# jlvdb/yet_another_wizz

Measured on AMD Instinct MI355X. Metric: candidate pairs/s, higher is better.
Workload: dtype f64

## Files before the change

yet_another_wizz_amd/csrc/yawhip_band32.inc:

```
namespace {

constexpr int B32_WAVES_PLAIN = 7;
constexpr int B32_WAVES_BIG = 6;
constexpr int B32_WAVES_W = 5;
constexpr int B32_WAVES_W1 = 5;
constexpr int B32_WAVES_LT = 1;
constexpr int band32_min_waves(int R, int CAP, bool WEIGHTED, int NE, bool UNI) {
    if (NE == 2 && UNI) {
        if (WEIGHTED) return R == 1 ? B32_WAVES_W1 : B32_WAVES_W;
        return CAP >= B32_CAP_BIG ? B32_WAVES_BIG : B32_WAVES_PLAIN;
    }
    return NE == 2 && !WEIGHTED ? B32_WAVES_LT : 1;
}

template <int R, int CAP, bool WEIGHTED, int NE, bool MERGED, bool UNI>
__global__ __launch_bounds__(64, band32_min_waves(R, CAP, WEIGHTED, NE, UNI))
void YAW_B32_NAME(const DevTab *__restrict__ tabs, const Item *__restrict__ items, int n_bins,
                  const double *__restrict__ t, const float *__restrict__ thr32,
                  const double *__restrict__ rwin_k, const float *__restrict__ ucap,
                  unsigned flush_mask, int swap,
                  unsigned long long *__restrict__ out_counts,
                  double *__restrict__ partials,
                  unsigned long long *__restrict__ counters, unsigned long long seg_cap) {
    static_assert(NE >= 2 && NE <= 4, "edges per bin");
    constexpr int CH = YAW_B32_CH;
    constexpr bool PAIRS = R == 1 && CH == 1;
    constexpr int NS = PAIRS ? 2 : R;
    static_assert(CH == 1 || CH == 3, "chunks per round");
    static_assert(CAP % 4 == 0, "stage capacity");
    using HistT = typename std::conditional<WEIGHTED, double, unsigned int>::type;
    constexpr int NC = NE == 2 ? 1 : NE;
    constexpr int NF = NE - 1;
    constexpr int TW = thr32_width(NE);
    constexpr bool LANE_THR = MERGED && !UNI;
    extern __shared__ __attribute__((aligned(16))) unsigned char lds_dyn[];
    const int nkb = MERGED ? n_bins : 1;
    const int nslots = nkb * NF;
    unsigned char *p = lds_dyn;
    constexpr unsigned COLB = (CAP + 4) * 4;
    float *stage = reinterpret_cast<float *>(p); p += (size_t)3 * COLB;
    double *sw = reinterpret_cast<double *>(p); if (WEIGHTED) p += (size_t)(CAP + 4) * 8;
    HistT *hist = reinterpret_cast<HistT *>(p); p += (size_t)nslots * sizeof(HistT);
    p = reinterpret_cast<unsigned char *>(((size_t)p + 15) & ~(size_t)15);
    float *sthr = reinterpret_cast<float *>(p);
    const int lane = threadIdx.x;
    const unsigned a_stage = (unsigned)(size_t)(lds_byte *)reinterpret_cast<unsigned char *>(stage);
    const unsigned a_sw = (unsigned)(size_t)(lds_byte *)reinterpret_cast<unsigned char *>(sw);
    const unsigned a_hist = (unsigned)(size_t)(lds_byte *)reinterpret_cast<unsigned char *>(hist);

    const TicketMap tmap = ticket_map(counters, seg_cap);
    const unsigned long long n_kept = tmap.n_kept;
    for (int e = lane; e < nslots; e += 64) hist[e] = HistT(0);
    if (LANE_THR)
        for (int e = lane; e < n_bins * TW; e += 64) sthr[e] = thr32[e];
    unsigned round_no = 0;
    for (unsigned long long v = blockIdx.x;; v += gridDim.x) {
        if ((v >> 3) >= tmap.per_xcd) break;
        const unsigned long long ticket = tmap.ticket(v);
        if (ticket >= n_kept) continue;
        const Item it = items[ticket];
        const int o = item_orient(it), islot = item_slot(it);
        const DevTab cl = tabs[swap ? o : 3 + o], cs = tabs[swap ? 3 + o : o];
        const int kfix = MERGED ? 0 : islot % n_bins;
        const float rwin = (float)(rwin_k[kfix] * 1.000001 + 4e-7);

        int win = 0;
        int64_t win_off = 0;
        int64_t cb[CH];
        int cn[CH], co[CH];
        int nch = 0;
        auto next_round = [&]() {
            nch = 0;
            int used = 0;
#pragma unroll
            for (int c = 0; c < CH; ++c) {
                cb[c] = 0; cn[c] = 0; co[c] = 0;
                if (win < it.nwin && nch == c) {
                    const int64_t wb = win == 0 ? it.b0[0] : (win == 1 ? it.b0[1] : it.b0[2]);
                    const int64_t rem = (int64_t)(win == 0 ? it.nb[0] : (win == 1 ? it.nb[1] : it.nb[2])) - win_off;
                    if (rem + 1 <= (int64_t)(CAP - used)) {
                        cb[c] = wb + win_off; cn[c] = (int)rem; co[c] = used;
                        used += ((int)rem + 1 + 3) & ~3;
                        ++win; win_off = 0; ++nch;
                    } else if (c == 0) {
                        cb[c] = wb + win_off; cn[c] = CAP - 4; co[c] = 0;
                        used = CAP;
                        win_off += CAP - 4; ++nch;
                    }
                }
            }
        };
        auto issue_round = [&]() {
#pragma unroll
            for (int c = 0; c < CH; ++c) {
                if (c < nch) {
                    const gf32p gx = cs.qx + cb[c], gy = cs.qy + cb[c], gz = cs.qz + cb[c];
                    const unsigned a_c = a_stage + ((unsigned)co[c] << 2);
#pragma unroll
                    for (int k = 0; k < (CAP + 255) / 256; ++k) {
                        const unsigned e = (unsigned)(k * 256 + 4 * lane);
                        if (e < (unsigned)cn[c]) {
                            __builtin_amdgcn_global_load_lds(gx + e, lds_ptr(a_c + k * 1024), 16, 0, 0);
                            __builtin_amdgcn_global_load_lds(gy + e, lds_ptr(a_c + COLB + k * 1024), 16, 0, 0);
                            __builtin_amdgcn_global_load_lds(gz + e, lds_ptr(a_c + 2 * COLB + k * 1024), 16, 0, 0);
                        }
                    }
                    if (WEIGHTED && cs.w) {
#pragma unroll
                        for (int k = 0; k < (CAP + 127) / 128; ++k) {
                            const unsigned e = (unsigned)(k * 128 + 2 * lane);
                            if (e < (unsigned)cn[c])
                                __builtin_amdgcn_global_load_lds(cs.w + cb[c] + e, lds_ptr(a_sw + ((unsigned)co[c] << 3) + k * 1024), 16, 0, 0);
                        }
                    }
                }
            }
        };
        __syncthreads();
        next_round();
        issue_round();
        f32x2 ax2[R / 2 > 0 ? R / 2 : 1], ay2[R / 2 > 0 ? R / 2 : 1], az2[R / 2 > 0 ? R / 2 : 1];
        float ax[R], ay[R], az[R];
        int kb[R];
        double aw_own[R];
        int lane_obj = lane;
        int n_own = (int)it.na - lane * R;
        n_own = n_own < 0 ? 0 : (n_own > R ? R : n_own);
#pragma unroll
        for (int r = 0; r < R; ++r) {
            const bool have = r < n_own;
            const unsigned ic = have ? (unsigned)(lane * R + r) : 0u;
            ax[r] = have ? (cl.qx + it.a0)[ic] : PAD_COORD32;
            ay[r] = have ? (cl.qy + it.a0)[ic] : PAD_COORD32;
            az[r] = have ? (cl.qz + it.a0)[ic] : PAD_COORD32;
            kb[r] = MERGED ? (have ? (cl.k + it.a0)[ic] : 0) : 0;
            if constexpr (WEIGHTED) aw_own[r] = (cl.w && have) ? (cl.w + it.a0)[ic] : 1.0;
        }
        float th[R][TW];
        {
            const float *row = LANE_THR ? nullptr : thr32 + (size_t)kfix * TW;
#pragma unroll
            for (int r = 0; r < R; ++r)
#pragma unroll
                for (int q = 0; q < TW; ++q) th[r][q] = LANE_THR ? sthr[kb[r] * TW + q] : row[q];
        }
        float klo, khi;
        {
            const int last_r = n_own > 0 ? n_own - 1 : 0;
            float u_first = cl.axis == 0 ? ax[0] : (cl.axis == 1 ? ay[0] : az[0]), u_last = u_first;
#pragma unroll
            for (int r = 1; r < R; ++r)
                if (r == last_r) u_last = cl.axis == 0 ? ax[r] : (cl.axis == 1 ? ay[r] : az[r]);
            klo = u_first - rwin;
            khi = u_last + rwin;
            const float cap_c = ucap[2 * kfix], cap_s = ucap[2 * kfix + 1];
            if (cap_s > 0.0f) {
                klo = cap_lo32(u_first, cap_c, cap_s);
                khi = cap_hi32(u_last, cap_c, cap_s);
            }
        }
        if constexpr (R >= 2) {
#pragma unroll
            for (int h = 0; h < R / 2; ++h) {
                ax2[h] = f32x2{ax[2 * h], ax[2 * h + 1]}; ay2[h] = f32x2{ay[2 * h], ay[2 * h + 1]}; az2[h] = f32x2{az[2 * h], az[2 * h + 1]};
            }
        }
        f32x2 nc2[R / 2 > 0 ? R / 2 : 1];
#pragma unroll
        for (int h = 0; h < R / 2; ++h) nc2[h] = f32x2{-th[2 * h][0], -th[2 * h + 1][0]};
        unsigned int cnt[R][NC];
        double acc[R][NC];
#pragma unroll
        for (int r = 0; r < R; ++r)
#pragma unroll
            for (int c = 0; c < NC; ++c) { cnt[r][c] = 0u; acc[r][c] = 0.0; }
        unsigned int nev = 0;
        constexpr bool HALF = R == 1 && CH == 1;
        const double pair_mult = HALF && (it.pad_ & 1) ? 2.0 : 1.0;
        auto flush_lanes = [&]() {
#pragma unroll
            for (int r = 0; r < R; ++r) {
#pragma unroll
                for (int f = 0; f < NF; ++f) {
                    const unsigned cell = a_hist + (unsigned)((kb[r] * NF + f) * (int)sizeof(HistT));
                    if constexpr (WEIGHTED) {
                        const double vsum = NE == 2 ? acc[r][0] : acc[r][f + 1] - acc[r][f];
                        const double aw = aw_own[r];
                        if (vsum != 0.0)
                            (void)__hip_atomic_fetch_add((__attribute__((address_space(3))) double *)(size_t)cell, HALF ? aw * vsum * pair_mult : aw * vsum,
                                                         __ATOMIC_RELAXED, __HIP_MEMORY_SCOPE_WORKGROUP);
                    } else {
                        const unsigned int c = (NE == 2 ? cnt[r][0] : cnt[r][f + 1] - cnt[r][f]) << (HALF ? (it.pad_ & 1) : 0);
                        if (c)
                            (void)__hip_atomic_fetch_add((__attribute__((address_space(3))) unsigned int *)(size_t)cell, c,
                                                         __ATOMIC_RELAXED, __HIP_MEMORY_SCOPE_WORKGROUP);
                    }
                }
#pragma unroll
                for (int c = 0; c < NC; ++c) { cnt[r][c] = 0u; acc[r][c] = 0.0; }
            }
        };
        auto flush_counts = [&]() {
            flush_lanes();
            __syncthreads();
            for (int idx = lane; idx < nslots; idx += 64) {
                const unsigned int c = (unsigned int)hist[idx];
                hist[idx] = HistT(0);
                if (c) atomicAdd(&out_counts[(int64_t)islot * nslots + idx], (unsigned long long)c);
            }
        };

        const bool single_window = it.nwin == 1 && it.nb[0] + 1 <= CAP;
        for (;; ++round_no) {
            asm volatile("s_waitcnt vmcnt(0)" ::: "memory");
            __syncthreads();
            if (lane < nch) {
                int at = co[0] + cn[0];
                if constexpr (CH > 1) at = lane == 0 ? at : (lane == 1 ? co[1] + cn[1] : co[CH - 1] + cn[CH - 1]);
                stage[at] = PAD_COORD32; stage[COLB / 4 + at] = PAD_COORD32; stage[2 * (COLB / 4) + at] = PAD_COORD32;
                if (WEIGHTED) sw[at] = 0.0;
                if constexpr (PAIRS) {
                    stage[at + 1] = PAD_COORD32; stage[COLB / 4 + at + 1] = PAD_COORD32; stage[2 * (COLB / 4) + at + 1] = PAD_COORD32;
                    if (WEIGHTED) sw[at + 1] = 0.0;
                }
            }
            if (WEIGHTED && !cs.w) {
#pragma unroll
                for (int c = 0; c < CH; ++c)
                    if (c < nch)
                        for (int e = lane; e < cn[c]; e += 64) sw[co[c] + e] = 1.0;
            }
            __syncthreads();
            unsigned a_key[CH], a_sent[CH], ql[CH], qh[CH];
            int n_max = 1;
#pragma unroll
            for (int c = 0; c < CH; ++c) {
                a_key[c] = a_stage + COLB * (unsigned)cl.axis + ((unsigned)co[c] << 2);
                a_sent[c] = a_key[c] + ((unsigned)cn[c] << 2);
                ql[c] = qh[c] = a_key[c] - 4u;
                n_max = cn[c] > n_max ? cn[c] : n_max;
            }
            for (unsigned step = 4u << (31 - __builtin_clz(n_max)); step >= 4u; step >>= 1) {
#pragma unroll
                for (int c = 0; c < CH; ++c) {
                    if (c < nch) {
                        const unsigned pl = ql[c] + step, ph = qh[c] + step;
                        const float kl = *(const __attribute__((address_space(3))) float *)(size_t)(pl < a_sent[c] ? pl : a_sent[c]);
                        const float kh = *(const __attribute__((address_space(3))) float *)(size_t)(ph < a_sent[c] ? ph : a_sent[c]);
                        ql[c] = kl < klo ? pl : ql[c];
                        qh[c] = kh <= khi ? ph : qh[c];
                    }
                }
            }
#pragma unroll
            for (int c = 0; c < CH; ++c) {
            if (c < nch) {
            const int n = cn[c];
            int lo = (int)((ql[c] + 4u - a_key[c]) >> 2), hi = (int)((qh[c] + 4u - a_key[c]) >> 2);
            if (n_own == 0) lo = hi = n;
            if constexpr (R == 1 && CH == 1) {
                if (it.pad_ & 1) {
                    const int own = n_own > 0 ? (int)((long long)(cl.pos3 + it.a0)[lane] - (long long)cb[c]) + 1 : n;
                    lo = own > lo ? own : lo;
                    lo = lo > hi ? hi : lo;
                }
            }
            int len = hi - lo;
            unsigned stride = PAIRS ? 8u : 4u;
            nev += (unsigned int)(len * n_own);
            if (single_window) {
                const unsigned long long act = __builtin_amdgcn_ballot_w64(len > 0);
                const int first = act ? __builtin_ctzll(act) : 0, span = act ? 64 - __builtin_clzll(act) - first : 64;
                if (span <= 32) {
                    const int sh = span <= 8 ? 3 : (span <= 16 ? 2 : 1);
                    const bool idle = (lane >> sh) >= span;
                    const int src = idle ? first : first + (lane >> sh);
                    const int part = lane & ((1 << sh) - 1);
                    if constexpr (R >= 2) {
#pragma unroll
                        for (int h = 0; h < R / 2; ++h) {
                            ax2[h] = f32x2{__shfl(ax2[h].x, src, 64), __shfl(ax2[h].y, src, 64)};
                            ay2[h] = f32x2{__shfl(ay2[h].x, src, 64), __shfl(ay2[h].y, src, 64)};
                            az2[h] = f32x2{__shfl(az2[h].x, src, 64), __shfl(az2[h].y, src, 64)};
                        }
                    }
#pragma unroll
                    for (int r = 0; r < R; ++r) {
                        if constexpr (R < 2) { ax[r] = __shfl(ax[r], src, 64); ay[r] = __shfl(ay[r], src, 64); az[r] = __shfl(az[r], src, 64); }
                        if constexpr (MERGED) kb[r] = __shfl(kb[r], src, 64);
                        if constexpr (WEIGHTED) aw_own[r] = __shfl(aw_own[r], src, 64);
                        if constexpr (LANE_THR) {
#pragma unroll
                            for (int q = 0; q < TW; ++q) th[r][q] = sthr[kb[r] * TW + q];
                        }
                    }
                    if constexpr (LANE_THR && NE == 2) {
#pragma unroll
                        for (int h = 0; h < R / 2; ++h) nc2[h] = f32x2{-th[2 * h][0], -th[2 * h + 1][0]};
                    }
                    n_own = __shfl(n_own, src, 64);
                    lane_obj = src;
                    const int lo_s = __shfl(lo, src, 64), len_s = __shfl(len, src, 64);
                    if constexpr (PAIRS) {
                        const int pairs_s = (len_s + 1) >> 1;
                        lo = idle ? n : lo_s + 2 * part;
                        len = !idle && pairs_s > part ? ((pairs_s - part + (1 << sh) - 1) >> sh) << 1 : 0;
                        stride = 8u << sh;
                    } else {
                        lo = idle ? n : lo_s + part;
                        len = !idle && len_s > part ? (len_s - part + (1 << sh) - 1) >> sh : 0;
                        stride = 4u << sh;
                    }
                }
            }
            const int steps = wave_max_nonneg(PAIRS ? (len + 1) >> 1 : len);

            const unsigned a_chunk = a_stage + ((unsigned)co[c] << 2);
            unsigned cur = a_chunk + ((unsigned)lo << 2);
            const unsigned last = a_chunk + ((unsigned)n << 2);
            auto eval_entry = [&](const unsigned a16) {
                struct { float x, y, z; } en, en1;
                en.x = *(const __attribute__((address_space(3))) float *)(size_t)a16;
                en.y = *(const __attribute__((address_space(3))) float *)(size_t)(a16 + COLB);
                en.z = *(const __attribute__((address_space(3))) float *)(size_t)(a16 + 2 * COLB);
                if constexpr (PAIRS) {
                    en1.x = *(const __attribute__((address_space(3))) float *)(size_t)(a16 + 4u);
                    en1.y = *(const __attribute__((address_space(3))) float *)(size_t)(a16 + 4u + COLB);
                    en1.z = *(const __attribute__((address_space(3))) float *)(size_t)(a16 + 4u + 2 * COLB);
                }
                double ewi[NS];
                const unsigned a_w = ((a16 - a_stage) << 1) + a_sw;
                ewi[0] = WEIGHTED ? lds_f64(a_w) : 1.0;
                if constexpr (PAIRS) ewi[1] = WEIGHTED ? lds_f64(a_w + 8u) : 1.0;
                else {
#pragma unroll
                    for (int i = 1; i < NS; ++i) ewi[i] = ewi[0];
                }
                float s32[NS];
                if constexpr (PAIRS) {
                    const f32x2 dx = ax[0] - f32x2{en.x, en1.x}, dy = ay[0] - f32x2{en.y, en1.y}, dz = az[0] - f32x2{en.z, en1.z};
                    f32x2 sq;
                    if constexpr (NE == 2) {
                        const f32x2 nc = f32x2{-th[0][0], -th[0][0]};
                        sq = __builtin_elementwise_fma(dz, dz, __builtin_elementwise_fma(dy, dy, __builtin_elementwise_fma(dx, dx, nc)));
                    } else sq = __builtin_elementwise_fma(dz, dz, __builtin_elementwise_fma(dy, dy, dx * dx));
                    s32[0] = sq.x; s32[1] = sq.y;
                } else if constexpr (R >= 2) {
#pragma unroll
                    for (int h = 0; h < R / 2; ++h) {
                        const f32x2 dx = ax2[h] - en.x, dy = ay2[h] - en.y, dz = az2[h] - en.z;
                        f32x2 sq;
                        if constexpr (NE == 2) sq = __builtin_elementwise_fma(dz, dz, __builtin_elementwise_fma(dy, dy, __builtin_elementwise_fma(dx, dx, nc2[h])));
                        else sq = __builtin_elementwise_fma(dz, dz, __builtin_elementwise_fma(dy, dy, dx * dx));
                        s32[2 * h] = sq.x; s32[2 * h + 1] = sq.y;
                    }
                } else {
                    const float dx = ax[0] - en.x, dy = ay[0] - en.y, dz = az[0] - en.z;
                    if constexpr (NE == 2) s32[0] = __builtin_fmaf(dz, dz, __builtin_fmaf(dy, dy, __builtin_fmaf(dx, dx, -th[0][0])));
                    else s32[0] = __builtin_fmaf(dz, dz, __builtin_fmaf(dy, dy, dx * dx));
                }
                unsigned long long unc_mask[NS];
                unsigned long long any_mask = 0ull;
#pragma unroll
                for (int i = 0; i < NS; ++i) {
                    const int r = PAIRS ? 0 : i;
                    const double ew = ewi[i];
                    if constexpr (NE == 2) {
                        const float q = __builtin_fabsf(s32[i]);
                        const bool in = q < th[r][1];
                        unc_mask[i] = __builtin_amdgcn_ballot_w64(q < th[r][2]) & ~__builtin_amdgcn_ballot_w64(in);
                        if constexpr (WEIGHTED) acc[r][0] = __builtin_fma(in ? 1.0 : 0.0, ew, acc[r][0]);
                        else cnt[r][0] += in ? 1u : 0u;
                    } else {
                        unc_mask[i] = 0ull;
#pragma unroll
                        for (int e = 0; e < NE; ++e) {
                            const bool le = s32[i] < th[r][2 * e];
                            unc_mask[i] |= __builtin_amdgcn_ballot_w64(s32[i] <= th[r][2 * e + 1]) & ~__builtin_amdgcn_ballot_w64(le);
                            if constexpr (WEIGHTED) acc[r][e] = __builtin_fma(le ? 1.0 : 0.0, ew, acc[r][e]);
                            else cnt[r][e] += le ? 1u : 0u;
                        }
                    }
                    any_mask |= unc_mask[i];
                }
                if (any_mask != 0ull) {
#pragma unroll
                    for (int i = 0; i < NS; ++i) {
                        const int r = PAIRS ? 0 : i;
                        const unsigned eidx = ((a16 - a_chunk) >> 2) + (PAIRS ? (unsigned)i : 0u);
                        const double ew = ewi[i];
                        if (((unc_mask[i] >> lane) & 1ull) && eidx < (unsigned)n && r < n_own) {
                            const ExactEval<NE> ev = band32_exact<NE>(cl.x, cl.y, cl.z, it.a0 + lane_obj * R + r, cs.x, cs.y, cs.z,
                                                                      cs.idx ? (int64_t)cs.idx[cb[c] + eidx] : cb[c] + (int64_t)eidx,
                                                                      t + (size_t)(MERGED ? kb[r] : kfix) * NE,
                                                                      counters + EXACT_EVAL_CTR(0) + CTR_SLOT_WORDS * (ticket & (EVAL_SLOTS - 1)));
                            const double sd = ev.s;
                            if constexpr (NE == 2) {
                                const bool in = sd > ev.th[0] && sd <= ev.th[1];
                                if constexpr (WEIGHTED) acc[r][0] += in ? ew : 0.0;
                                else cnt[r][0] += in ? 1u : 0u;
                            } else {
#pragma unroll
                                for (int e = 0; e < NE; ++e) {
                                    const bool open = !(s32[i] < th[r][2 * e]) && s32[i] <= th[r][2 * e + 1];
                                    const bool le = open && sd <= ev.th[e];
                                    if constexpr (WEIGHTED) acc[r][e] += le ? ew : 0.0;
                                    else cnt[r][e] += le ? 1u : 0u;
                                }
                            }
                        }
                    }
                }
            };
            constexpr int UNROLL = 1;
            for (int s = 0; s < steps; s += UNROLL) {
#pragma unroll
                for (int uu = 0; uu < UNROLL; ++uu) {
                    const unsigned at = cur + stride * (unsigned)uu;
                    eval_entry(at < last ? at : last);
                }
                cur += stride * UNROLL;
            }
            }
            }
            if (!WEIGHTED && (round_no & flush_mask) == flush_mask) flush_counts();
            if (win >= it.nwin) break;
            __syncthreads();
            next_round();
            issue_round();
        }
        ++round_no;
        if constexpr (WEIGHTED) {
            flush_lanes();
            __syncthreads();
            for (int idx = lane; idx < nslots; idx += 64) {
                partials[(int64_t)it.pot * nslots + idx] = (double)hist[idx];
                hist[idx] = HistT(0);
            }
        } else {
            flush_counts();
        }
        nev = wave_sum_lane63(nev);
        if (lane == 63 && nev) atomicAdd(&counters[BAND_ENTRY_CTR(ticket & (EVAL_SLOTS - 1))], (unsigned long long)nev);
    }
}

}

namespace yawhip_detail {

hipError_t YAW_B32_LAUNCH(const CountLaunch &L, bool wgt, int32_t *variant) {
    const std::pair<int, int> stage{L.R, L.cap};
    const std::pair<bool, bool> rows{L.merged, L.uni};
    const dim3 band_grid(L.band_grid), wave(64);
    return pick<Bool<false>, Bool<true>>(wgt, [&](auto w) {
        return pick<Int<4>, Int<3>, Int<2>>(L.n_edges, [&](auto ne) {
            return pick<Rows<true, false>, Rows<true, true>, Rows<false, true>>(rows, [&](auto r) {
                return pick<Stage<4, B32_CAP_BIG>, Stage<2, B32_CAP_BIG>, Stage<2, B32_CAP>, Stage<1, B32_CAP>>(stage, [&](auto s) {
                    using S = decltype(s);
                    using M = decltype(r);
                    *variant = variant_code(YAW_B32_CH == 1 ? VF_BAND32_ONE : VF_BAND32, S::R, S::CAP, w, ne, M::MERGED, M::UNI);
                    return launch(YAW_B32_NAME<S::R, S::CAP, w, ne, M::MERGED, M::UNI>, band_grid, wave, L.lds, L.stream, L.d_tabs,
                                  L.d_items, L.n_bins, L.d_t, L.d_thr32, L.d_rwin, L.d_ucap, L.flush_mask, L.swap ? 1 : 0,
                                  L.d_counts, L.d_partials, L.d_ctr, L.seg_cap);
                });
            });
        });
    });
}

}
```

yet_another_wizz_amd/csrc/yawhip_count_kernels.h:

```cpp
#ifndef YAWHIP_COUNT_KERNELS_H
#define YAWHIP_COUNT_KERNELS_H
#include <hip/hip_runtime.h>

#include <algorithm>
#include <cmath>
#include <cstddef>
#include <cstdint>

#include "yawhip_internal.h"

#pragma GCC visibility push(hidden)

namespace yawhip_detail {

constexpr int WG = 256;
constexpr int STAGE = 256;
constexpr int MSTAGE = 64;
constexpr int MAX_EDGES = 512;
constexpr int BAND_MIN_STREAM_RUN = 64;
constexpr int64_t SYNC_GRID_MIN_ITEMS = 400000;
constexpr int MAX_STRIP_REACH = 12;

constexpr double FILTER_GUARD = 8.0 * 5.9604644775390625e-8;

inline double sep_angle(double rwin) { return 2.0 * std::asin(std::min(1.0, 0.5 * (rwin + 2e-9))); }

constexpr int EVAL_SLOTS = 256;
constexpr int BUILD_WG = 1024;
constexpr int BUILD_WG_SMALL = 256;
inline int build_wg_for(int64_t n_pot) { return n_pot / 256 <= 4096 ? BUILD_WG_SMALL : BUILD_WG; }
constexpr int BUILD_PREFIX_LDS = 1024;
constexpr int ITEM_SEGS = 8;

constexpr int BCAP = 192;
constexpr int BCAP_MID = 288;
constexpr int B32_CAP = 320;
constexpr int B32_CAP_BIG = 512;

constexpr double BAND32_GUARD_SQRT = 2.1e-7;
__host__ __device__ constexpr int thr32_width(int ne) { return ne == 2 ? 4 : 2 * ne; }
__host__ __device__ constexpr int fine32_width(int n_edges) { return 4 + 2 * n_edges; }

constexpr int REDUCE_CHUNK = 32;
constexpr int TAIL_WG = 256;
constexpr unsigned TAIL_MAX_GRID = 64;
constexpr double CLOCK_MS = 1.0e-5;

int band_lds_fixed(int cap);
__host__ __device__ inline bool band_small_hist(bool weighted, int nslots, int hp) { return (size_t)nslots * hp * (weighted ? 8 : 4) <= 512; }
__host__ __device__ inline size_t band_lds_dynamic(bool weighted, bool need_thr, int nkb, int n_edges, int hp, int cap, int thr_rows) {
    const int nslots = nkb * (n_edges - 1);
    return (weighted ? (size_t)(cap + 2) * 8 : 0) + (need_thr ? (size_t)thr_rows * n_edges * sizeof(double) : 0) +
           (band_small_hist(weighted, nslots, hp) ? 0 : (size_t)nslots * hp * (weighted ? 8 : 4)) + 16;
}
__host__ __device__ inline size_t band32_lds(bool weighted, int cap, int nslots, int thr_rows, int ne) {
    return (size_t)3 * (cap + 4) * 4 + (weighted ? (size_t)(cap + 4) * 8 : 0) + (size_t)nslots * (weighted ? 8 : 4) +
           (size_t)thr_rows * thr32_width(ne) * 4 + 32;
}
__host__ __device__ inline size_t band32_fine_lds(bool weighted, int cap, int nslots, int rows, int n_edges) {
    return (size_t)3 * (cap + 4) * 4 + (weighted ? (size_t)(cap + 2) * 8 : 0) + (size_t)nslots * (weighted ? 8 : 4) + 64 * 8 +
           (size_t)rows * fine32_width(n_edges) * 4 + 48;
}
size_t count_lds(bool weighted, bool priv, int n_edges);
size_t merged_stage_lds();
size_t merged_lds(bool weighted, int bins, int n_edges);

constexpr int CTR_KEPT = 0, CTR_T_BUILD = 1, CTR_T_COUNTED = 2, CTR_T_TAIL = 3, CTR_TICKET = 4, CTR_DONE = 6;
constexpr int CTR_SLOT_WORDS = 8;
template <typename I> __host__ __device__ constexpr auto BAND_ENTRY_CTR(I i) { return 8 + CTR_SLOT_WORDS * i; }
template <typename I> __host__ __device__ constexpr auto EXACT_EVAL_CTR(I i) { return 9 + CTR_SLOT_WORDS * i; }
template <typename I> __host__ __device__ constexpr auto TILE_PAIR_CTR(I i) { return 10 + CTR_SLOT_WORDS * i; }
__host__ __device__ constexpr int ITEM_SEG_CTR(int seg) { return 12 + CTR_SLOT_WORDS * seg; }
__host__ __device__ constexpr int SEG_EXIT_CTR(int seg) { return ITEM_SEG_CTR(seg) + 1; }
constexpr int N_CTR = 8 + CTR_SLOT_WORDS * EVAL_SLOTS;
static_assert(BAND_ENTRY_CTR(0) % CTR_SLOT_WORDS == 0 && EXACT_EVAL_CTR(0) % CTR_SLOT_WORDS == 1 && TILE_PAIR_CTR(0) % CTR_SLOT_WORDS == 2 &&
                  ITEM_SEG_CTR(0) % CTR_SLOT_WORDS == 4 && SEG_EXIT_CTR(0) % CTR_SLOT_WORDS == 5,
              "the segment words and the per-slot words take different places of a slot's line");
static_assert(CTR_DONE < BAND_ENTRY_CTR(0) && ITEM_SEGS <= EVAL_SLOTS && TILE_PAIR_CTR(EVAL_SLOTS - 1) < N_CTR, "counter block");

enum class CountFamily : int32_t { PLAIN, LEAN, BAND64, BAND32, BAND32_FINE };
struct CountLaunch {
    hipStream_t stream = nullptr;
    CountFamily family = CountFamily::PLAIN;
    int R = 0, cap = 0, band_ne = 0;
    bool merged = false, uni = false, nf1 = false, filter = false, priv = false, one_chunk = false;
    unsigned build_grid = 0, build_wg = 0, band_grid = 0;
    int64_t n_pot = 0;
    int64_t n_items = 0;
    int64_t n_build_jobs = 0;
    int64_t n_oslots = 0;
    int64_t tile = 0, slab = 0, n_chunks = 0;
    size_t lds = 0;
    unsigned flush_mask = 0;
    int batch_log2 = 0, hp_shift = 0, n_bins = 0, n_edges = 0, reach = 0;
    bool swap = false, triple = false;
    unsigned long long seg_cap = 0;
    double rwin_max = 0.0, cap_c = 1.0, cap_s = 0.0;
    CatView c1{}, c2{};
    const DevTab *d_tabs = nullptr;
    const int32_t *d_jobs = nullptr;
    const int64_t *d_prefix = nullptr, *d_cprefix = nullptr;
    const double *d_t = nullptr, *d_rwin = nullptr;
    const float *d_dthr = nullptr, *d_ucap = nullptr, *d_thr32 = nullptr;
    Item *d_items = nullptr;
    unsigned char *d_kept = nullptr;
    unsigned long long *d_ctr = nullptr, *d_counts = nullptr;
    double *d_partials = nullptr, *d_chunk_sums = nullptr, *d_sums = nullptr;
};

hipError_t launch_build_strips(const CountLaunch &L);
hipError_t launch_build_windows(const CountLaunch &L);
hipError_t launch_build_whole(const CountLaunch &L);
hipError_t launch_item_work(const CountLaunch &L, int slots_per_job, unsigned long long *job_work);
hipError_t launch_count(const CountLaunch &L, bool weighted, int32_t *variant);
hipError_t launch_plain(const CountLaunch &L, bool weighted, int32_t *variant);
hipError_t launch_lean(const CountLaunch &L, bool weighted, int32_t *variant);
hipError_t launch_band64(const CountLaunch &L, bool weighted, int32_t *variant);
hipError_t launch_band32(const CountLaunch &L, bool weighted, int32_t *variant);
hipError_t launch_band32_one(const CountLaunch &L, bool weighted, int32_t *variant);
hipError_t launch_fine(const CountLaunch &L, bool weighted, int32_t *variant);
hipError_t launch_reduce_chunks(const CountLaunch &L);
hipError_t launch_reduce_slots(const CountLaunch &L);
hipError_t launch_counts_to_double(const CountLaunch &L, int64_t n_out);
hipError_t launch_call_tail(hipStream_t stream, unsigned char *dev, unsigned char *host, unsigned n_copy, unsigned n_clean,
                            unsigned long long seq);

}

#pragma GCC visibility pop
#endif
```

Measured before the change: 34220000 billion.

## Hand-code unweighted two-slot band32 inner loop in packed-f32 inline asm

For unweighted two-edge, two-object (R=2) band32 kernels without per-lane thresholds, the per-entry classify step is replaced by inline assembly. It uses packed f32 subtract/FMA, scalar-mask comparisons and carry-add counting, and splits classification from the rare exact-evaluation path. When there is one chunk per round, the loop walks the staged entries downward from the top using a clamped subtract. It pads four leading LDS slots with PAD_COORD32 so out-of-range reads hit sentinels, and reserves 48 extra LDS bytes for this. The goal is fewer VALU/SALU instructions and less loop-control overhead per candidate. The cost is brittle asm, a trap if the LDS base is not the expected offset, and more LDS use.

```diff
diff --git a/yet_another_wizz_amd/csrc/yawhip_band32.inc b/yet_another_wizz_amd/csrc/yawhip_band32.inc
--- a/yet_another_wizz_amd/csrc/yawhip_band32.inc
+++ b/yet_another_wizz_amd/csrc/yawhip_band32.inc
@@ -37,8 +37,12 @@
     const int nkb = MERGED ? n_bins : 1;
     const int nslots = nkb * NF;
     unsigned char *p = lds_dyn;
-    constexpr unsigned COLB = (CAP + 4) * 4;
-    float *stage = reinterpret_cast<float *>(p); p += (size_t)3 * COLB;
+    constexpr bool SLOT_TRIP = NE == 2 && !WEIGHTED && R == 2 && !LANE_THR;
+    constexpr bool DOWN = SLOT_TRIP && CH == 1;
+    constexpr int LEAD = DOWN ? 4 : 0;
+    constexpr unsigned COLB = (CAP + 4 + LEAD) * 4;
+    float *const stage_lead = reinterpret_cast<float *>(p);
+    float *stage = stage_lead + LEAD; p += (size_t)3 * COLB;
     double *sw = reinterpret_cast<double *>(p); if (WEIGHTED) p += (size_t)(CAP + 4) * 8;
     HistT *hist = reinterpret_cast<HistT *>(p); p += (size_t)nslots * sizeof(HistT);
     p = reinterpret_cast<unsigned char *>(((size_t)p + 15) & ~(size_t)15);
@@ -51,6 +55,10 @@
     const TicketMap tmap = ticket_map(counters, seg_cap);
     const unsigned long long n_kept = tmap.n_kept;
     for (int e = lane; e < nslots; e += 64) hist[e] = HistT(0);
+    if constexpr (DOWN) {
+        if (a_stage != 4u * LEAD) __builtin_trap();
+        if (lane < LEAD) { stage_lead[lane] = PAD_COORD32; stage_lead[COLB / 4 + lane] = PAD_COORD32; stage_lead[2 * (COLB / 4) + lane] = PAD_COORD32; }
+    }
     if (LANE_THR)
         for (int e = lane; e < n_bins * TW; e += 64) sthr[e] = thr32[e];
     unsigned round_no = 0;
@@ -266,6 +274,7 @@
                 }
             }
             int len = hi - lo;
+            int top = hi - 1;
             unsigned stride = PAIRS ? 8u : 4u;
             nev += (unsigned int)(len * n_own);
             if (single_window) {
@@ -308,6 +317,7 @@
                         stride = 8u << sh;
                     } else {
                         lo = idle ? n : lo_s + part;
+                        top = lo_s + len_s - 1 - part;
                         len = !idle && len_s > part ? (len_s - part + (1 << sh) - 1) >> sh : 0;
                         stride = 4u << sh;
                     }
@@ -318,7 +328,7 @@
             const unsigned a_chunk = a_stage + ((unsigned)co[c] << 2);
             unsigned cur = a_chunk + ((unsigned)lo << 2);
             const unsigned last = a_chunk + ((unsigned)n << 2);
-            auto eval_entry = [&](const unsigned a16) {
+            auto classify_entry = [&](const unsigned a16, unsigned long long (&unc_mask)[NS], float (&s32)[NS], double (&ewi)[NS]) {
                 struct { float x, y, z; } en, en1;
                 en.x = *(const __attribute__((address_space(3))) float *)(size_t)a16;
                 en.y = *(const __attribute__((address_space(3))) float *)(size_t)(a16 + COLB);
@@ -328,7 +338,6 @@
                     en1.y = *(const __attribute__((address_space(3))) float *)(size_t)(a16 + 4u + COLB);
                     en1.z = *(const __attribute__((address_space(3))) float *)(size_t)(a16 + 4u + 2 * COLB);
                 }
-                double ewi[NS];
                 const unsigned a_w = ((a16 - a_stage) << 1) + a_sw;
                 ewi[0] = WEIGHTED ? lds_f64(a_w) : 1.0;
                 if constexpr (PAIRS) ewi[1] = WEIGHTED ? lds_f64(a_w + 8u) : 1.0;
@@ -336,7 +345,6 @@
 #pragma unroll
                     for (int i = 1; i < NS; ++i) ewi[i] = ewi[0];
                 }
-                float s32[NS];
                 if constexpr (PAIRS) {
                     const f32x2 dx = ax[0] - f32x2{en.x, en1.x}, dy = ay[0] - f32x2{en.y, en1.y}, dz = az[0] - f32x2{en.z, en1.z};
                     f32x2 sq;
@@ -359,7 +367,6 @@
                     if constexpr (NE == 2) s32[0] = __builtin_fmaf(dz, dz, __builtin_fmaf(dy, dy, __builtin_fmaf(dx, dx, -th[0][0])));
                     else s32[0] = __builtin_fmaf(dz, dz, __builtin_fmaf(dy, dy, dx * dx));
                 }
-                unsigned long long unc_mask[NS];
                 unsigned long long any_mask = 0ull;
 #pragma unroll
                 for (int i = 0; i < NS; ++i) {
@@ -383,43 +390,119 @@
                     }
                     any_mask |= unc_mask[i];
                 }
-                if (any_mask != 0ull) {
-#pragma unroll
-                    for (int i = 0; i < NS; ++i) {
-                        const int r = PAIRS ? 0 : i;
-                        const unsigned eidx = ((a16 - a_chunk) >> 2) + (PAIRS ? (unsigned)i : 0u);
-                        const double ew = ewi[i];
-                        if (((unc_mask[i] >> lane) & 1ull) && eidx < (unsigned)n && r < n_own) {
-                            const ExactEval<NE> ev = band32_exact<NE>(cl.x, cl.y, cl.z, it.a0 + lane_obj * R + r, cs.x, cs.y, cs.z,
-                                                                      cs.idx ? (int64_t)cs.idx[cb[c] + eidx] : cb[c] + (int64_t)eidx,
-                                                                      t + (size_t)(MERGED ? kb[r] : kfix) * NE,
-                                                                      counters + EXACT_EVAL_CTR(0) + CTR_SLOT_WORDS * (ticket & (EVAL_SLOTS - 1)));
-                            const double sd = ev.s;
-                            if constexpr (NE == 2) {
-                                const bool in = sd > ev.th[0] && sd <= ev.th[1];
-                                if constexpr (WEIGHTED) acc[r][0] += in ? ew : 0.0;
-                                else cnt[r][0] += in ? 1u : 0u;
-                            } else {
-#pragma unroll
-                                for (int e = 0; e < NE; ++e) {
-                                    const bool open = !(s32[i] < th[r][2 * e]) && s32[i] <= th[r][2 * e + 1];
-                                    const bool le = open && sd <= ev.th[e];
-                                    if constexpr (WEIGHTED) acc[r][e] += le ? ew : 0.0;
-                                    else cnt[r][e] += le ? 1u : 0u;
-                                }
+                return any_mask;
+            };
+            auto classify_two_objects = [&](unsigned &a16, unsigned &cur_, int &rem, unsigned long long (&unc_mask)[NS]) {
+                if constexpr (!SLOT_TRIP) return 0ull;
+                else {
+                f32x2 ex, ey, ez, q, dy, dz;
+                ex.x = *(const __attribute__((address_space(3))) float *)(size_t)a16;
+                ey.x = *(const __attribute__((address_space(3))) float *)(size_t)(a16 + COLB);
+                ez.x = *(const __attribute__((address_space(3))) float *)(size_t)(a16 + 2 * COLB);
+                unsigned long long in1, any_mask;
+#define YAW_TRIP_SUMS_(slot)                                                                          \
+    "v_pk_add_f32 v[0:1], %[ax], %[ex] op_sel_hi:[1,0] neg_lo:[0,1] neg_hi:[0,1]\n\t"                   \
+    "v_pk_add_f32 %[dy], %[ay], %[ey] op_sel_hi:[1,0] neg_lo:[0,1] neg_hi:[0,1]\n\t"                    \
+    "v_pk_fma_f32 v[0:1], v[0:1], v[0:1], %[nc]\n\t"                                                    \
+    "v_pk_add_f32 %[dz], %[az], %[ez] op_sel_hi:[1,0] neg_lo:[0,1] neg_hi:[0,1]\n\t"                    \
+    "v_pk_fma_f32 v[0:1], %[dy], %[dy], v[0:1]\n\t" slot "\n\t"                                        \
+    "v_pk_fma_f32 v[0:1], %[dz], %[dz], v[0:1]\n\t"
+#define YAW_TRIP_CLASSES_                                     \
+    "v_cmp_lt_f32_e64 vcc, |v0|, %[hin]\n\t"                  \
+    "v_cmp_lt_f32_e64 %[in1], |v1|, %[hin]\n\t"               \
+    "v_cmp_lt_f32_e64 %[u0], |v0|, %[hout]\n\t"               \
+    "v_cmp_lt_f32_e64 %[u1], |v1|, %[hout]\n\t"               \
+    "s_andn2_b64 %[u0], %[u0], vcc\n\t"                       \
+    "s_andn2_b64 %[u1], %[u1], %[in1]\n\t"                    \
+    "v_addc_co_u32_e64 %[c0], vcc, 0, %[c0], vcc\n\t"         \
+    "v_addc_co_u32_e64 %[c1], %[in1], 0, %[c1], %[in1]\n\t"   \
+    "s_or_b64 %[any], %[u0], %[u1]"
+                if constexpr (DOWN) {
+                    asm volatile(YAW_TRIP_SUMS_("v_sub_u32_e64 %[a], %[a], %[stride] clamp") "s_add_i32 %[rem], %[rem], -1\n\t" YAW_TRIP_CLASSES_
+                                 : [q] "=&{v[0:1]}"(q), [dy] "=&v"(dy), [dz] "=&v"(dz), [a] "+v"(a16), [rem] "+s"(rem),
+                                   [in1] "=&s"(in1), [u0] "=&s"(unc_mask[0]), [u1] "=&s"(unc_mask[1]), [any] "=&s"(any_mask),
+                                   [c0] "+v"(cnt[0][0]), [c1] "+v"(cnt[1][0])
+                                 : [ax] "v"(ax2[0]), [ay] "v"(ay2[0]), [az] "v"(az2[0]), [ex] "v"(ex), [ey] "v"(ey), [ez] "v"(ez),
+                                   [nc] "s"(nc2[0]), [stride] "s"(stride), [hin] "s"(th[0][1]), [hout] "s"(th[0][2])
+                                 : "vcc", "scc");
+                } else {
+                    asm volatile(YAW_TRIP_SUMS_("v_add_u32 %[cur], %[stride], %[cur]") "v_min_u32 %[nxt], %[last], %[cur]\n\t" YAW_TRIP_CLASSES_
+                                 : [q] "=&{v[0:1]}"(q), [dy] "=&v"(dy), [dz] "=&v"(dz), [cur] "+v"(cur_), [nxt] "=&v"(a16),
+                                   [in1] "=&s"(in1), [u0] "=&s"(unc_mask[0]), [u1] "=&s"(unc_mask[1]), [any] "=&s"(any_mask),
+                                   [c0] "+v"(cnt[0][0]), [c1] "+v"(cnt[1][0])
+                                 : [ax] "v"(ax2[0]), [ay] "v"(ay2[0]), [az] "v"(az2[0]), [ex] "v"(ex), [ey] "v"(ey), [ez] "v"(ez),
+                                   [nc] "s"(nc2[0]), [stride] "s"(stride), [last] "s"(last), [hin] "s"(th[0][1]), [hout] "s"(th[0][2])
+                                 : "vcc", "scc");
+                }
+#undef YAW_TRIP_SUMS_
+#undef YAW_TRIP_CLASSES_
+                return any_mask;
+                }
+            };
+            auto settle_entry = [&](const unsigned a16, const unsigned long long (&unc_mask)[NS], const float (&s32)[NS], const double (&ewi)[NS]) {
+#pragma unroll
+                for (int i = 0; i < NS; ++i) {
+                    const int r = PAIRS ? 0 : i;
+                    const unsigned eidx = ((a16 - a_chunk) >> 2) + (PAIRS ? (unsigned)i : 0u);
+                    const double ew = ewi[i];
+                    if (((unc_mask[i] >> lane) & 1ull) && eidx < (unsigned)n && r < n_own) {
+                        const ExactEval<NE> ev = band32_exact<NE>(cl.x, cl.y, cl.z, it.a0 + lane_obj * R + r, cs.x, cs.y, cs.z,
+                                                                  cs.idx ? (int64_t)cs.idx[cb[c] + eidx] : cb[c] + (int64_t)eidx,
+                                                                  t + (size_t)(MERGED ? kb[r] : kfix) * NE,
+                                                                  counters + EXACT_EVAL_CTR(0) + CTR_SLOT_WORDS * (ticket & (EVAL_SLOTS - 1)));
+                        const double sd = ev.s;
+                        if constexpr (NE == 2) {
+                            const bool in = sd > ev.th[0] && sd <= ev.th[1];
+                            if constexpr (WEIGHTED) acc[r][0] += in ? ew : 0.0;
+                            else cnt[r][0] += in ? 1u : 0u;
+                        } else {
+#pragma unroll
+                            for (int e = 0; e < NE; ++e) {
+                                const bool open = !(s32[i] < th[r][2 * e]) && s32[i] <= th[r][2 * e + 1];
+                                const bool le = open && sd <= ev.th[e];
+                                if constexpr (WEIGHTED) acc[r][e] += le ? ew : 0.0;
+                                else cnt[r][e] += le ? 1u : 0u;
                             }
                         }
                     }
                 }
             };
-            constexpr int UNROLL = 1;
-            for (int s = 0; s < steps; s += UNROLL) {
-#pragma unroll
-                for (int uu = 0; uu < UNROLL; ++uu) {
-                    const unsigned at = cur + stride * (unsigned)uu;
-                    eval_entry(at < last ? at : last);
-                }
-                cur += stride * UNROLL;
+            if constexpr (DOWN) {
+                const unsigned start = len > 0 ? a_chunk + ((unsigned)top << 2) : 0u;
+                unsigned a16 = start, unused = 0u;
+                int rem = steps;
+                while (rem != 0) {
+                    unsigned long long unc_mask[NS];
+                    if (__builtin_expect(classify_two_objects(a16, unused, rem, unc_mask) != 0ull, 0)) {
+                        const float s32[NS] = {0.0f, 0.0f};
+                        const double ewi[NS] = {1.0, 1.0};
+                        const unsigned back = (unsigned)(steps - rem - 1) * stride;
+                        settle_entry(start > back ? start - back : 0u, unc_mask, s32, ewi);
+                    }
+                }
+            } else if constexpr (SLOT_TRIP) {
+                unsigned a16 = cur < last ? cur : last;
+                int unused = 0;
+                for (int s = 0; s < steps; ++s) {
+                    unsigned long long unc_mask[NS];
+                    if (__builtin_expect(classify_two_objects(a16, cur, unused, unc_mask) != 0ull, 0)) {
+                        const float s32[NS] = {0.0f, 0.0f};
+                        const double ewi[NS] = {1.0, 1.0};
+                        const unsigned at = cur - stride;
+                        settle_entry(at < last ? at : last, unc_mask, s32, ewi);
+                    }
+                }
+            } else {
+                auto eval_entry = [&](const unsigned a16) {
+                    unsigned long long unc_mask[NS];
+                    float s32[NS];
+                    double ewi[NS];
+                    if (__builtin_expect(classify_entry(a16, unc_mask, s32, ewi) != 0ull, 0)) settle_entry(a16, unc_mask, s32, ewi);
+                };
+                for (int s = 0; s < steps; ++s) {
+                    eval_entry(cur < last ? cur : last);
+                    cur += stride;
+                }
             }
             }
             }
diff --git a/yet_another_wizz_amd/csrc/yawhip_count_kernels.h b/yet_another_wizz_amd/csrc/yawhip_count_kernels.h
--- a/yet_another_wizz_amd/csrc/yawhip_count_kernels.h
+++ b/yet_another_wizz_amd/csrc/yawhip_count_kernels.h
@@ -55,7 +55,7 @@
 }
 __host__ __device__ inline size_t band32_lds(bool weighted, int cap, int nslots, int thr_rows, int ne) {
     return (size_t)3 * (cap + 4) * 4 + (weighted ? (size_t)(cap + 4) * 8 : 0) + (size_t)nslots * (weighted ? 8 : 4) +
-           (size_t)thr_rows * thr32_width(ne) * 4 + 32;
+           (size_t)thr_rows * thr32_width(ne) * 4 + 32 + (!weighted && ne == 2 && thr_rows == 0 ? 48 : 0);
 }
 __host__ __device__ inline size_t band32_fine_lds(bool weighted, int cap, int nslots, int rows, int n_edges) {
     return (size_t)3 * (cap + 4) * 4 + (weighted ? (size_t)(cap + 2) * 8 : 0) + (size_t)nslots * (weighted ? 8 : 4) + 64 * 8 +
```

Result: faster. 35500000 billion (median of 6 runs) (+3.8%).
